# hmmlillian/Neural-Color-Transfer

Measured on AMD Instinct MI355X. Metric: 700x700 pairs/sec end-to-end L=5->1; PatchMatch HBM GB/s vs peak, higher is better.
Workload: dtype f32

## Files before the change

### neural-color-transfer_amd/csrc/k_s1.hip

```cpp
#include "nct_internal.h"
#include "nct_device.h"
#include "nct_reduce.h"
#include <cstdlib>
#include <rocprim/device/device_radix_sort.hpp>
#include <rocprim/device/device_scan.hpp>

#define LAB_D(u) ((double)(u) * (1.0 / 255.0))
#define LCHK() NCT_LAUNCH_CHECK()

constexpr int S1_SEG = NCT_S1_SEG;

struct S1Sys {
    int n, h, w;
    const double *daa, *dab, *dbb;
    const double *gx, *gy;
    const int* knn_id;
    nct_s1_graph g;
    int xcd;
    int one_xcd;
};
__device__ __forceinline__ int s1_one_xcd(int bid, int sel) { return (bid & 7) == sel - 1 ? (bid >> 3) : -1; }
__device__ __forceinline__ int s1_block_of(int bid, int nblocks, int xcd) {
    if (!xcd) return bid;
    const int q = nblocks >> 3, r = nblocks & 7, x = bid & 7, idx = bid >> 3;
    return (x < r ? x * (q + 1) : r * (q + 1) + (x - r) * q) + idx;
}
struct S1State { double gm[3], al[3], be[3]; int active[3], iters[3]; };

__device__ __forceinline__ void ld6(const double* __restrict__ v, size_t px, double (&o)[6]) {
    const double2* q = reinterpret_cast<const double2*>(v + px * 6);
    const double2 t0 = q[0], t1 = q[1], t2 = q[2];
    o[0] = t0.x; o[1] = t0.y; o[2] = t1.x; o[3] = t1.y; o[4] = t2.x; o[5] = t2.y;
}
__device__ __forceinline__ void st6(double* __restrict__ v, size_t px, const double (&o)[6]) {
    double2* q = reinterpret_cast<double2*>(v + px * 6);
    q[0] = make_double2(o[0], o[1]); q[1] = make_double2(o[2], o[3]); q[2] = make_double2(o[4], o[5]);
}
__device__ __forceinline__ int lo32(unsigned long long v) { return (int)(unsigned)(v & 0xFFFFFFFFull); }
__device__ __forceinline__ int hi32(unsigned long long v) { return (int)(unsigned)(v >> 32); }

__global__ void k_s1_iw2(const double* __restrict__ knn_w, int m, double nonlocalWeight, double* __restrict__ iw2) {
    const int e = blockIdx.x * blockDim.x + threadIdx.x;
    if (e >= m) return;
    const double iw = sqrt(knn_w[e]) * nonlocalWeight;
    iw2[e] = iw * iw;
}
__global__ void k_edge_keys(const int* __restrict__ knn_id, int m, unsigned* __restrict__ keys, unsigned* __restrict__ vals) {
    const int e = blockIdx.x * blockDim.x + threadIdx.x;
    if (e >= m) return;
    keys[e] = (unsigned)knn_id[e]; vals[e] = (unsigned)e;
}
__global__ void k_seg_starts(const unsigned* __restrict__ keys, int m, int* __restrict__ start, int n) {
    const int s = blockIdx.x * blockDim.x + threadIdx.x;
    if (s > n) return;
    int lo = 0, hi = m;
    while (lo < hi) { const int mid = (lo + hi) >> 1; if (keys[mid] < (unsigned)s) lo = mid + 1; else hi = mid; }
    start[s] = lo;
}
__global__ void k_s1_counts(const int* __restrict__ rev_start, int n, unsigned long long* __restrict__ cnt) {
    const int i = blockIdx.x * blockDim.x + threadIdx.x;
    if (i > n) return;
    unsigned long long v = 0;
    if (i < n) {
        const int deg = rev_start[i + 1] - rev_start[i];
        v = (unsigned long long)(deg < S1_SEG ? deg : S1_SEG) | ((unsigned long long)(deg > S1_SEG ? (deg - 1) / S1_SEG : 0) << 32);
    }
    cnt[i] = v;
}
__global__ void k_s1_sup_counts(const unsigned long long* __restrict__ starts, int n, int* __restrict__ cnt) {
    const int i = blockIdx.x * blockDim.x + threadIdx.x;
    if (i > n) return;
    int c = 0;
    if (i < n) { const int m = hi32(starts[i + 1]) - hi32(starts[i]); c = m > S1_SEG ? (m + S1_SEG - 1) / S1_SEG : 0; }
    cnt[i] = c;
}
__global__ void k_s1_sup_fill(const unsigned long long* __restrict__ starts, const int* __restrict__ sup_start, int n, int* __restrict__ sup_b0) {
    const int i = blockIdx.x * blockDim.x + threadIdx.x;
    if (i >= n) return;
    const int s0 = sup_start[i], ns = sup_start[i + 1] - s0, b0 = hi32(starts[i]);
    for (int k = 0; k < ns; ++k) sup_b0[s0 + k] = b0 + k * S1_SEG;
}
__global__ void k_s1_rev_build(const unsigned* __restrict__ keys_sorted, const unsigned* __restrict__ edge_sorted, const double* __restrict__ iw2, int m,
                               const int* __restrict__ rev_start, const unsigned long long* __restrict__ starts,
                               int* __restrict__ c_src, double* __restrict__ c_w, int* __restrict__ rev_src, double* __restrict__ rev_w,
                               int* __restrict__ seg_tgt, int* __restrict__ seg_e0) {
    const int e = blockIdx.x * blockDim.x + threadIdx.x;
    if (e >= m) return;
    const int t = (int)keys_sorted[e];
    const int rank = e - rev_start[t];
    const unsigned ed = edge_sorted[e];
    const int src = (int)(ed >> 3); const double wt = iw2[ed];
    const unsigned long long st = starts[t];
    if (rank < S1_SEG) { const int pos = lo32(st) + rank; c_src[pos] = src; c_w[pos] = wt; }
    else {
        rev_src[e] = src; rev_w[e] = wt;
        if ((rank & (S1_SEG - 1)) == 0) { const int sg = hi32(st) + rank / S1_SEG - 1; seg_tgt[sg] = t; seg_e0[sg] = e; }
    }
}

int nctk_s1_graph_build(nct_ctx* ctx, hipStream_t s, const int* knn_id, const double* knn_w, double nonlocalWeight, const nct_s1_graph& g, int* nseg_pinned) {
    const int n = g.n, m = 8 * n;
    DevBuf<unsigned> ek(ctx, m), ev(ctx, m), eks(ctx, m), evs(ctx, m);
    DevBuf<unsigned long long> cnt(ctx, (size_t)n + 1);
    DevBuf<int> scnt(ctx, (size_t)n + 1);
    if (!ek.ok() || !ev.ok() || !eks.ok() || !evs.ok() || !cnt.ok() || !scnt.ok()) return NCT_ERR_HIP;
    hipLaunchKernelGGL(k_s1_iw2, dim3(cdiv(m, 256)), dim3(256), 0, s, knn_w, m, nonlocalWeight, g.iw2); LCHK();
    hipLaunchKernelGGL(k_edge_keys, dim3(cdiv(m, 256)), dim3(256), 0, s, knn_id, m, (unsigned*)ek, (unsigned*)ev); LCHK();
    int end_bit = 1; while ((1u << end_bit) < (unsigned)n && end_bit < 32) ++end_bit;
    size_t tmp_bytes = 0, scan_bytes = 0, scan2_bytes = 0;
    NCT_HIP(rocprim::radix_sort_pairs(nullptr, tmp_bytes, (const unsigned*)ek, (unsigned*)eks, (const unsigned*)ev, (unsigned*)evs, m, 0, end_bit, s));
    NCT_HIP(rocprim::exclusive_scan(nullptr, scan_bytes, (const unsigned long long*)cnt, g.starts, 0ull, (size_t)n + 1, rocprim::plus<unsigned long long>(), s));
    NCT_HIP(rocprim::exclusive_scan(nullptr, scan2_bytes, (const int*)scnt, g.sup_start, 0, (size_t)n + 1, rocprim::plus<int>(), s));
    if (scan2_bytes > scan_bytes) scan_bytes = scan2_bytes;
    DevBuf<char> tmp(ctx, (tmp_bytes > scan_bytes ? tmp_bytes : scan_bytes) + 16);
    if (!tmp.ok()) return NCT_ERR_HIP;
    NCT_HIP(rocprim::radix_sort_pairs((void*)(char*)tmp, tmp_bytes, (const unsigned*)ek, (unsigned*)eks, (const unsigned*)ev, (unsigned*)evs, m, 0, end_bit, s));
    hipLaunchKernelGGL(k_seg_starts, dim3(cdiv(n + 1, 256)), dim3(256), 0, s, (const unsigned*)eks, m, g.rev_start, n); LCHK();
    hipLaunchKernelGGL(k_s1_counts, dim3(cdiv(n + 1, 256)), dim3(256), 0, s, (const int*)g.rev_start, n, (unsigned long long*)cnt); LCHK();
    NCT_HIP(rocprim::exclusive_scan((void*)(char*)tmp, scan_bytes, (const unsigned long long*)cnt, g.starts, 0ull, (size_t)n + 1, rocprim::plus<unsigned long long>(), s));
    hipLaunchKernelGGL(k_s1_rev_build, dim3(cdiv(m, 256)), dim3(256), 0, s, (const unsigned*)eks, (const unsigned*)evs, (const double*)g.iw2, m, (const int*)g.rev_start,
                       (const unsigned long long*)g.starts, g.c_src, g.c_w, g.rev_src, g.rev_w, g.seg_tgt, g.seg_e0); LCHK();
    hipLaunchKernelGGL(k_s1_sup_counts, dim3(cdiv(n + 1, 256)), dim3(256), 0, s, (const unsigned long long*)g.starts, n, (int*)scnt); LCHK();
    NCT_HIP(rocprim::exclusive_scan((void*)(char*)tmp, scan2_bytes, (const int*)scnt, g.sup_start, 0, (size_t)n + 1, rocprim::plus<int>(), s));
    hipLaunchKernelGGL(k_s1_sup_fill, dim3(cdiv(n, 256)), dim3(256), 0, s, (const unsigned long long*)g.starts, (const int*)g.sup_start, n, g.sup_b0); LCHK();
    if (nseg_pinned) {
        NCT_HIP(hipMemcpyAsync(nseg_pinned, (const char*)(g.starts + n) + 4, sizeof(int), hipMemcpyDeviceToHost, s));
        NCT_HIP(hipMemcpyAsync(nseg_pinned + 1, g.sup_start + n, sizeof(int), hipMemcpyDeviceToHost, s));
    }
    return 0;
}

__global__ void k_s1_setup(int n, const double* __restrict__ weight, float dWeight, const uint8_t* __restrict__ src, const uint8_t* __restrict__ ref,
                           double* __restrict__ daa, double* __restrict__ dab, double* __restrict__ dbb, double* __restrict__ rhs ) {
    const int i = blockIdx.x * blockDim.x + threadIdx.x;
    if (i >= n) return;
    const double dw = sqrt(weight[i]) * (double)sqrtf(dWeight);
#pragma unroll
    for (int c = 0; c < 3; ++c) {
        const double v0 = dw * LAB_D(src[(size_t)i * 3 + c]);
        const double rb = dw * LAB_D(ref[(size_t)i * 3 + c]);
        daa[(size_t)i * 3 + c] = v0 * v0; dab[(size_t)i * 3 + c] = v0 * dw; dbb[(size_t)i * 3 + c] = dw * dw;
        rhs[(size_t)i * 3 + c] = v0 * rb; rhs[(size_t)(n + i) * 3 + c] = dw * rb;
    }
}

__global__ __launch_bounds__(256) void k_s1_hub(nct_s1_graph G, const double* __restrict__ v ) {
    const int nseg = hi32(G.starts[G.n]);
    const int lane = threadIdx.x & 63;
    for (int sg = blockIdx.x * 4 + (threadIdx.x >> 6); sg < nseg; sg += gridDim.x * 4) {
        const int t = G.seg_tgt[sg];
        const int e = G.seg_e0[sg] + lane;
        const bool in = e < G.rev_start[t + 1];
        double term[6], vt[6], vj[6];
        int j = t; double wt = 0.0;
        if (in) { j = G.rev_src[e]; wt = G.rev_w[e]; }
        ld6(v, (size_t)t, vt); ld6(v, (size_t)j, vj);
#pragma unroll
        for (int c = 0; c < 6; ++c) { const double d = wt * (vt[c] - vj[c]); term[c] = in ? d : 0.0; }
#pragma unroll
        for (int off = 32; off >= 1; off >>= 1)
#pragma unroll
            for (int c = 0; c < 6; ++c) term[c] += __shfl_xor(term[c], off);
        if (lane == 0) {
#pragma unroll
            for (int c = 0; c < 6; ++c) G.hub_part[(size_t)sg * 6 + c] = term[c];
        }
    }
}

__global__ __launch_bounds__(256) void k_s1_hub2(nct_s1_graph G) {
    const int nsup = G.sup_start[G.n];
    const int lane = threadIdx.x & 63;
    for (int sb = blockIdx.x * 4 + (threadIdx.x >> 6); sb < nsup; sb += gridDim.x * 4) {
        const int b0 = G.sup_b0[sb];
        const int t = G.seg_tgt[b0];
        const int bend = min(b0 + S1_SEG, hi32(G.starts[t + 1]));
        double term[6];
        const bool in = b0 + lane < bend;
        if (in) ld6(G.hub_part, (size_t)(b0 + lane), term);
#pragma unroll
        for (int c = 0; c < 6; ++c) term[c] = in ? term[c] : 0.0;
#pragma unroll
        for (int off = 32; off >= 1; off >>= 1)
#pragma unroll
            for (int c = 0; c < 6; ++c) term[c] += __shfl_xor(term[c], off);
        if (lane == 0) st6(G.sup_part, (size_t)sb, term);
    }
}

#ifndef NCT_S1_CHUNK
#define NCT_S1_CHUNK 1024
#endif
constexpr int S1_CHUNK = NCT_S1_CHUNK;
template <bool COOP>
__device__ __forceinline__ void s1_op(const S1Sys& S, const double* __restrict__ p, int i, bool live, double (&a)[3], double (&b)[3], double (&ya)[3], double (&yb)[3], int lb = -1) {
    const int w = S.w, h = S.h;
    int e0 = 0, e1 = 0, h0 = 0, h1 = 0;
#pragma unroll
    for (int c = 0; c < 3; ++c) { a[c] = 0.0; b[c] = 0.0; ya[c] = 0.0; yb[c] = 0.0; }
    if (live) {
        const int y = i / w, x = i - y * w;
        { double own[6]; ld6(p, (size_t)i, own);
#pragma unroll
          for (int c = 0; c < 3; ++c) { a[c] = own[c]; b[c] = own[3 + c]; } }
#pragma unroll
        for (int c = 0; c < 3; ++c) {
            ya[c] = S.daa[(size_t)i * 3 + c] * a[c] + S.dab[(size_t)i * 3 + c] * b[c];
            yb[c] = S.dab[(size_t)i * 3 + c] * a[c] + S.dbb[(size_t)i * 3 + c] * b[c];
        }
        auto edge = [&](int j, double wt) {
            double q[6]; ld6(p, (size_t)j, q);
#pragma unroll
            for (int c = 0; c < 3; ++c) { ya[c] += wt * (a[c] - q[c]); yb[c] += wt * (b[c] - q[3 + c]); }
        };
        {
            const bool ex[4] = {x + 1 < w, x > 0, y + 1 < h, y > 0};
            const int nj[4] = {ex[0] ? i + 1 : i, ex[1] ? i - 1 : i, ex[2] ? i + w : i, ex[3] ? i - w : i};
            const double g4[4] = {S.gx[i], S.gx[ex[1] ? i - 1 : i], S.gy[i], S.gy[ex[3] ? i - w : i]};
            double q4[4][6];
#pragma unroll
            for (int u = 0; u < 4; ++u) ld6(p, (size_t)nj[u], q4[u]);
#pragma unroll
            for (int u = 0; u < 4; ++u)
                if (ex[u]) {
                    const double wt = 2.0 * (g4[u] * g4[u]);
#pragma unroll
                    for (int c = 0; c < 3; ++c) { ya[c] += wt * (a[c] - q4[u][c]); yb[c] += wt * (b[c] - q4[u][3 + c]); }
                }
        }
#pragma unroll
        for (int k = 0; k < 8; ++k) edge(S.knn_id[(size_t)i * 8 + k], S.g.iw2[(size_t)i * 8 + k]);
        const unsigned long long s0 = S.g.starts[i], s1 = S.g.starts[i + 1];
        e0 = lo32(s0); e1 = lo32(s1); h0 = hi32(s0); h1 = hi32(s1);
    }
    if constexpr (!COOP) {
        if (live) {
            int e = e0;
            for (; e + 4 <= e1; e += 4) {
                int j[4]; double wt[4], pv[4][6];
#pragma unroll
                for (int u = 0; u < 4; ++u) { j[u] = S.g.c_src[e + u]; wt[u] = S.g.c_w[e + u]; }
#pragma unroll
                for (int u = 0; u < 4; ++u) ld6(p, (size_t)j[u], pv[u]);
#pragma unroll
                for (int u = 0; u < 4; ++u)
#pragma unroll
                    for (int c = 0; c < 3; ++c) { ya[c] += wt[u] * (a[c] - pv[u][c]); yb[c] += wt[u] * (b[c] - pv[u][3 + c]); }
            }
            for (; e < e1; ++e) {
                const int j = S.g.c_src[e]; const double wt = S.g.c_w[e];
                double q[6]; ld6(p, (size_t)j, q);
#pragma unroll
                for (int c = 0; c < 3; ++c) { ya[c] += wt * (a[c] - q[c]); yb[c] += wt * (b[c] - q[3 + c]); }
            }
        }
    } else {
        __shared__ double s_pv[6 * S1_CHUNK];
        __shared__ double s_wt[S1_CHUNK];
        const int i0 = (lb >= 0 ? lb : (int)blockIdx.x) * 256, i1 = min(i0 + 256, S.n);
        const int E0 = lo32(S.g.starts[i0]), E1 = lo32(S.g.starts[i1]);
        for (int base = E0; base < E1; base += S1_CHUNK) {
            const int cnt = min(S1_CHUNK, E1 - base);
            for (int t = threadIdx.x; t < cnt; t += 256) {
                const int j = S.g.c_src[base + t];
                s_wt[t] = S.g.c_w[base + t];
                double q[6]; ld6(p, (size_t)j, q);
#pragma unroll
                for (int c = 0; c < 6; ++c) s_pv[c * S1_CHUNK + t] = q[c];
            }
            __syncthreads();
            const int lo = max(e0, base) - base, hi = min(e1, base + cnt) - base;
            for (int t = lo; t < hi; ++t) {
                const double wt = s_wt[t];
#pragma unroll
                for (int c = 0; c < 3; ++c) { ya[c] += wt * (a[c] - s_pv[c * S1_CHUNK + t]); yb[c] += wt * (b[c] - s_pv[(3 + c) * S1_CHUNK + t]); }
            }
            __syncthreads();
        }
    }
    bool sup = false;
    if (h1 - h0 > S1_SEG) { h0 = S.g.sup_start[i]; h1 = S.g.sup_start[i + 1]; sup = true; }
    const double* __restrict__ part = sup ? S.g.sup_part : S.g.hub_part;
    for (int sg = h0; sg < h1; ++sg) {
        double q[6]; ld6(part, (size_t)sg, q);
#pragma unroll
        for (int c = 0; c < 3; ++c) { ya[c] += q[c]; yb[c] += q[3 + c]; }
    }
}

template <bool COOP>
__global__ __launch_bounds__(256) void k_s1_residual(S1Sys S, const double* __restrict__ x6, const double* __restrict__ rhs, double* __restrict__ r6) {
    const int i = blockIdx.x * 256 + threadIdx.x;
    double a[3], b[3], ya[3], yb[3];
    s1_op<COOP>(S, x6, i, i < S.n, a, b, ya, yb);
    if (i < S.n) {
        double o[6];
#pragma unroll
        for (int c = 0; c < 3; ++c) { o[c] = rhs[(size_t)i * 3 + c] - ya[c]; o[3 + c] = rhs[(size_t)(S.n + i) * 3 + c] - yb[c]; }
        st6(r6, (size_t)i, o);
    }
}
template <bool COOP>
__global__ __launch_bounds__(256) void k_s1_apply(S1Sys S, const double* __restrict__ r6, double* __restrict__ w6, double* __restrict__ partial ) {
    const int lb = S.one_xcd ? s1_one_xcd(blockIdx.x, S.one_xcd) : s1_block_of(blockIdx.x, gridDim.x, S.xcd);
    if (lb < 0) return;
    const int i = lb * 256 + threadIdx.x;
    double acc[6] = {0, 0, 0, 0, 0, 0};
    double a[3], b[3], ya[3], yb[3];
    s1_op<COOP>(S, r6, i, i < S.n, a, b, ya, yb, lb);
    if (i < S.n) {
#pragma unroll
        for (int c = 0; c < 3; ++c) {
            acc[c] = a[c] * a[c] + b[c] * b[c];
            acc[3 + c] = a[c] * ya[c] + b[c] * yb[c];
        }
        const double o[6] = {ya[0], ya[1], ya[2], yb[0], yb[1], yb[2]};
        st6(w6, (size_t)i, o);
    }
    block_reduce_store<6>(acc, partial, lb);
}

__device__ __forceinline__ void s1_scalars(bool first, const double (&sm)[6], const S1State* __restrict__ in, double tol2, S1State& o) {
#pragma unroll
    for (int c = 0; c < 3; ++c) {
        if (first) {
            const double g0 = sm[c]; const bool act = g0 > tol2;
            o.gm[c] = g0; o.be[c] = 0.0; o.al[c] = act ? g0 / sm[3 + c] : 0.0; o.active[c] = act ? 1 : 0; o.iters[c] = act ? 1 : 0;
        } else if (in->active[c]) {
            const double g1 = sm[c];
            const double be = g1 / in->gm[c];
            const double al = g1 / (sm[3 + c] - (be * g1) / in->al[c]);
            const bool act = g1 > tol2;
            o.gm[c] = g1; o.be[c] = be; o.al[c] = al; o.active[c] = act ? 1 : 0; o.iters[c] = in->iters[c] + (act ? 1 : 0);
        } else {
            o.gm[c] = in->gm[c]; o.be[c] = in->be[c]; o.al[c] = in->al[c]; o.active[c] = 0; o.iters[c] = in->iters[c];
        }
    }
}
__global__ __launch_bounds__(256) void k_s1_scal(const double* __restrict__ partial, int nb, const S1State* __restrict__ in, S1State* __restrict__ out, int first, double tol2) {
    double sm[6]; final_reduce<6>(partial, nb, sm);
    if (threadIdx.x == 0) { S1State o; s1_scalars(first != 0, sm, in, tol2, o); *out = o; }
}
constexpr int S1_FUSE_NB = 512;
template <bool FUSED>
__global__ __launch_bounds__(256) void k_s1_update(int n, int nb, const double* __restrict__ partial, const S1State* __restrict__ sin, S1State* __restrict__ sout,
                                                   int first_scal, double tol2, int first_vec, double* __restrict__ r6, const double* __restrict__ w6,
                                                   double* __restrict__ p6, double* __restrict__ s6, double* __restrict__ x6, int one_xcd) {
    const int bid = one_xcd ? s1_one_xcd(blockIdx.x, one_xcd) : (int)blockIdx.x;
    if (bid < 0) return;
    const size_t total = (size_t)3 * n;
    const size_t base = (size_t)bid * 768 + threadIdx.x;
    double2 rv[3], wv[3], pv[3], sv[3], xv[3];
    const double2* r2 = reinterpret_cast<const double2*>(r6); const double2* w2 = reinterpret_cast<const double2*>(w6);
    const double2* x2 = reinterpret_cast<const double2*>(x6); const double2* p2 = reinterpret_cast<const double2*>(p6); const double2* s2 = reinterpret_cast<const double2*>(s6);
#pragma unroll
    for (int k = 0; k < 3; ++k) {
        const size_t g0 = base + (size_t)k * 256, g = g0 < total ? g0 : total - 1;
        rv[k] = r2[g]; wv[k] = w2[g]; xv[k] = x2[g];
        pv[k] = p2[g]; sv[k] = s2[g];
        if (first_vec) { pv[k] = make_double2(0.0, 0.0); sv[k] = make_double2(0.0, 0.0); }
    }
    double al[3], be[3]; bool act[3];
    if constexpr (FUSED) {
        double sm[6]; final_reduce<6>(partial, nb, sm);
        S1State o; s1_scalars(first_scal != 0, sm, sin, tol2, o);
        if (bid == 0 && threadIdx.x == 0) *sout = o;
#pragma unroll
        for (int c = 0; c < 3; ++c) { al[c] = o.al[c]; be[c] = o.be[c]; act[c] = o.active[c] != 0; }
    } else {
#pragma unroll
        for (int c = 0; c < 3; ++c) { al[c] = sin->al[c]; be[c] = sin->be[c]; act[c] = sin->active[c] != 0; }
    }
    double2* r2o = reinterpret_cast<double2*>(r6); double2* x2o = reinterpret_cast<double2*>(x6); double2* p2o = reinterpret_cast<double2*>(p6); double2* s2o = reinterpret_cast<double2*>(s6);
#pragma unroll
    for (int k = 0; k < 3; ++k) {
        const size_t g = base + (size_t)k * 256;
        if (g >= total) continue;
        const int c0 = (int)((2 * g) % 3), c1 = (c0 + 1) % 3;
        const double a0 = c0 == 0 ? al[0] : (c0 == 1 ? al[1] : al[2]), b0 = c0 == 0 ? be[0] : (c0 == 1 ? be[1] : be[2]);
        const double a1 = c1 == 0 ? al[0] : (c1 == 1 ? al[1] : al[2]), b1 = c1 == 0 ? be[0] : (c1 == 1 ? be[1] : be[2]);
        const bool on0 = c0 == 0 ? act[0] : (c0 == 1 ? act[1] : act[2]), on1 = c1 == 0 ? act[0] : (c1 == 1 ? act[1] : act[2]);
        double2 pn, sn, xn, rn;
        pn.x = first_vec ? rv[k].x : b0 * pv[k].x + rv[k].x;  pn.y = first_vec ? rv[k].y : b1 * pv[k].y + rv[k].y;
        sn.x = first_vec ? wv[k].x : b0 * sv[k].x + wv[k].x;  sn.y = first_vec ? wv[k].y : b1 * sv[k].y + wv[k].y;
        xn.x = xv[k].x + a0 * pn.x;  xn.y = xv[k].y + a1 * pn.y;
        rn.x = rv[k].x - a0 * sn.x;  rn.y = rv[k].y - a1 * sn.y;
        if (!on0) { pn.x = pv[k].x; sn.x = sv[k].x; xn.x = xv[k].x; rn.x = rv[k].x; }
        if (!on1) { pn.y = pv[k].y; sn.y = sv[k].y; xn.y = xv[k].y; rn.y = rv[k].y; }
        if (on0 || on1) { p2o[g] = pn; s2o[g] = sn; x2o[g] = xn; r2o[g] = rn; }
    }
}
__global__ void k_pack6(int n, const double* __restrict__ x, double* __restrict__ x6) {
    const int i = blockIdx.x * blockDim.x + threadIdx.x;
    if (i >= 2 * n * 3) return;
    const int c = i % 3, part = i / (n * 3), px = (i - part * n * 3) / 3;
    x6[(size_t)px * 6 + part * 3 + c] = x[i];
}
__global__ void k_unpack6(int n, const double* __restrict__ x6, double* __restrict__ x) {
    const int i = blockIdx.x * blockDim.x + threadIdx.x;
    if (i >= 2 * n * 3) return;
    const int c = i % 3, part = i / (n * 3), px = (i - part * n * 3) / 3;
    x[i] = x6[(size_t)px * 6 + part * 3 + c];
}

int nctk_s1_solve(nct_ctx* ctx, hipStream_t s, const nct_s1_graph& g, const int* knn_id, const double* weight, float dWeight, const uint8_t* s_lab_level,
                  const uint8_t* g_lab_level, const double* gx, const double* gy, int layer, int h, int w, double* x, int* cg_iters_host ) {
    const int n = h * w, nbl = cdiv(n, 256);
    DevBuf<double> daa(ctx, (size_t)3 * n), dab(ctx, (size_t)3 * n), dbb(ctx, (size_t)3 * n), rhs(ctx, (size_t)6 * n);
    DevBuf<double> x6(ctx, (size_t)6 * n), r6(ctx, (size_t)6 * n), w6(ctx, (size_t)6 * n), p6(ctx, (size_t)6 * n), s6(ctx, (size_t)6 * n), partial(ctx, (size_t)nbl * 6);
    DevBuf<S1State> st(ctx, 2);
    if (!daa.ok() || !dab.ok() || !dbb.ok() || !rhs.ok() || !x6.ok() || !r6.ok() || !w6.ok() || !p6.ok() || !s6.ok() || !partial.ok() || !st.ok()) return NCT_ERR_HIP;
    hipLaunchKernelGGL(k_s1_setup, dim3(nbl), dim3(256), 0, s, n, weight, dWeight, s_lab_level, g_lab_level, (double*)daa, (double*)dab, (double*)dbb, (double*)rhs); LCHK();
    static const int s1_xcd = [] { const char* e = getenv("NCT_S1_XCD"); return e ? atoi(e) : 1; }();
    static const int s1_one_max = [] { const char* e = getenv("NCT_S1_ONE_XCD_MAX"); return e ? atoi(e) : 32; }();
    const int one_xcd = (nbl <= s1_one_max && nbl <= S1_FUSE_NB) ? 1 + (ctx->home_xcd & 7) : 0;
    const int ogrid = one_xcd ? nbl * 8 : nbl;
    S1Sys S{n, h, w, daa, dab, dbb, gx, gy, knn_id, g, (s1_xcd && n >= 100000) ? 1 : 0, one_xcd};
    const double tol2 = 1e-6 * 1e-6;
    const int maxit = layer == 4 ? 50 : 100;
    const bool coop = n >= 100000;
    const bool fused = nbl <= S1_FUSE_NB;
    const int hub_blind = cdiv(cdiv(8 * n, S1_SEG), 4) < 256 ? cdiv(cdiv(8 * n, S1_SEG), 4) : 256;
    const int hub_grid = g.nseg_hint == 0 ? 0 : (g.nseg_hint > 0 ? (cdiv(g.nseg_hint, 4) < 4096 ? cdiv(g.nseg_hint, 4) : 4096) : hub_blind);
    const int hub2_grid = (g.nseg_hint == 0 || g.nsup_hint == 0) ? 0 : (g.nsup_hint > 0 ? (cdiv(g.nsup_hint, 4) < 1024 ? cdiv(g.nsup_hint, 4) : 1024) : (cdiv(hub_blind, S1_SEG) < 64 ? cdiv(hub_blind, S1_SEG) : 64));
    auto hub = [&](const double* v) -> int {
        if (hub_grid) { hipLaunchKernelGGL(k_s1_hub, dim3(hub_grid), dim3(256), 0, s, g, v); LCHK(); }
        if (hub2_grid) { hipLaunchKernelGGL(k_s1_hub2, dim3(hub2_grid), dim3(256), 0, s, g); LCHK(); }
        return 0;
    };
    auto apply = [&](bool kt) -> int {
        if (kt) { int rk = ctx->kt_begin(s, NCT_KT_S1_APPLY); if (rk) return rk; }
        if (coop) hipLaunchKernelGGL(k_s1_apply<true>, dim3(nbl), dim3(256), 0, s, S, (const double*)r6, (double*)w6, (double*)partial);
        else      hipLaunchKernelGGL(k_s1_apply<false>, dim3(ogrid), dim3(256), 0, s, S, (const double*)r6, (double*)w6, (double*)partial);
        LCHK();
        if (kt) { int rk = ctx->kt_end(s); if (rk) return rk; }
        return 0;
    };
    hipLaunchKernelGGL(k_pack6, dim3(cdiv(6 * n, 256)), dim3(256), 0, s, n, (const double*)x, (double*)x6); LCHK();
    { int rc = hub(x6); if (rc) return rc; }
    if (coop) hipLaunchKernelGGL(k_s1_residual<true>, dim3(nbl), dim3(256), 0, s, S, (const double*)x6, (const double*)rhs, (double*)r6);
    else      hipLaunchKernelGGL(k_s1_residual<false>, dim3(nbl), dim3(256), 0, s, S, (const double*)x6, (const double*)rhs, (double*)r6);
    LCHK();
    { int rc = hub(r6); if (rc) return rc; rc = apply(false); if (rc) return rc; }
    S1State* slot[2] = {(S1State*)st, (S1State*)st + 1};
    for (int k = 1; k <= maxit; ++k) {
        const bool kt = ctx->kt_on && layer == 4 && k >= 3 && k < 11;
        if (fused) {
            hipLaunchKernelGGL(k_s1_update<true>, dim3(ogrid), dim3(256), 0, s, n, nbl, (const double*)partial, (const S1State*)slot[k & 1], slot[(k - 1) & 1], k == 1 ? 1 : 0, tol2,
                               k == 1 ? 1 : 0, (double*)r6, (const double*)w6, (double*)p6, (double*)s6, (double*)x6, one_xcd); LCHK();
        } else {
            if (kt) { int rk = ctx->kt_begin(s, NCT_KT_S1_SCALARS); if (rk) return rk; }
            hipLaunchKernelGGL(k_s1_scal, dim3(1), dim3(256), 0, s, (const double*)partial, nbl, (const S1State*)slot[k & 1], slot[(k - 1) & 1], k == 1 ? 1 : 0, tol2); LCHK();
            if (kt) { int rk = ctx->kt_end(s); if (rk) return rk; rk = ctx->kt_begin(s, NCT_KT_S1_UPDATE); if (rk) return rk; }
            hipLaunchKernelGGL(k_s1_update<false>, dim3(nbl), dim3(256), 0, s, n, nbl, (const double*)partial, (const S1State*)slot[(k - 1) & 1], slot[(k - 1) & 1], 0, tol2,
                               k == 1 ? 1 : 0, (double*)r6, (const double*)w6, (double*)p6, (double*)s6, (double*)x6, 0); LCHK();
            if (kt) { int rk = ctx->kt_end(s); if (rk) return rk; }
        }
        if (k < maxit) { int rc = hub(r6); if (rc) return rc; rc = apply(kt); if (rc) return rc; }
    }
    hipLaunchKernelGGL(k_unpack6, dim3(cdiv(6 * n, 256)), dim3(256), 0, s, n, (const double*)x6, x); LCHK();
    if (cg_iters_host) {
        S1State hst;
        NCT_HIP(hipMemcpyAsync(&hst, slot[(maxit - 1) & 1], sizeof hst, hipMemcpyDeviceToHost, s));
        NCT_HIP(hipStreamSynchronize(s));
        for (int c = 0; c < 3; ++c) cg_iters_host[c] = hst.iters[c];
    }
    return 0;
}
```

### neural-color-transfer_amd/csrc/nct_internal.h

```cpp
#pragma once
#include <hip/hip_runtime.h>
#include <cstdint>
#include <cstdio>
#include <cstdarg>
#include <string>
#include <vector>
#include "../../include/nct.h"

struct nct_block { void* p; size_t bytes; bool used; };

struct nct_ctx {
    int device = 0;
    hipStream_t stream = nullptr;
    hipStream_t stream2 = nullptr;
    hipEvent_t ev0 = nullptr, ev1 = nullptr, ev_fork = nullptr, ev_join = nullptr;
    hipEvent_t ev_level[5] = {nullptr, nullptr, nullptr, nullptr, nullptr};
    hipEvent_t ev_poll[4] = {nullptr, nullptr, nullptr, nullptr};
    hipStream_t stream_wls = nullptr;
    hipEvent_t ev_wls_fork = nullptr, ev_wls_join = nullptr;
    void* pinned = nullptr;
    std::string err;
    std::vector<nct_block> blocks;
    size_t bytes_allocated = 0;
    float *bench_a = nullptr, *bench_b = nullptr; void *bench_ah16 = nullptr, *bench_bh16 = nullptr; int bench_C = 0, bench_ah = 0, bench_aw = 0, bench_bh = 0, bench_bw = 0;
    void* vgg = nullptr;
    void* cvt = nullptr;
    void* pair = nullptr;
    unsigned long long* d_counter = nullptr;
    int home_xcd = 0;
    int pm_persist = 0;
    int pm_persist_wgs = 0;
    uint32_t* d_pm_err = nullptr;
    unsigned pm_attr_mask = 0;
    int wls_split = 0;
    int wls_forecast = 1;
    int wls_lines = 1;
    int wls_graph = 0;
    int conv_pool_fuse = -1;
    double wls_rtol = 3e-8;
    int wls_maxit = 5000;
    bool tm_on = false;
    std::vector<hipEvent_t> tm_events;
    std::vector<double> tm_host;
    std::vector<int> tm_tags;
    int mark(hipStream_t s, int tag);
    int conv_pair = 1;
    int* s1_hub_blocks() { return (int*)((char*)pinned + 4096); }
    long long s1_hub_blocks_last[5] = {0, 0, 0, 0, 0};
    int knn_runs = -1;
    int s1_hub_hint = 1;
    int s1_hub_wait = 1;
    bool kt_on = false;
    std::vector<hipEvent_t> kt_events; std::vector<int> kt_ids;
    int kt_begin(hipStream_t s, int id);
    int kt_end(hipStream_t s);

    int fail(int code, const char* fmt, ...) {
        char buf[512]; va_list ap; va_start(ap, fmt); vsnprintf(buf, sizeof buf, fmt, ap); va_end(ap);
        err = buf; return code;
    }
    void* alloc(size_t bytes);
    void release(void* p);
    bool defer_release = false;
    std::vector<void*> deferred;
    void flush_deferred() { for (void* p : deferred) for (auto& b : blocks) if (b.p == p) { b.used = false; break; } deferred.clear(); }
};

template <typename T> struct DevBuf {
    nct_ctx* c; T* p;
    DevBuf(nct_ctx* ctx, size_t n) : c(ctx), p((T*)ctx->alloc(n * sizeof(T))) {}
    ~DevBuf() { if (p) c->release(p); }
    DevBuf(const DevBuf&) = delete; DevBuf& operator=(const DevBuf&) = delete;
    operator T*() const { return p; }
    bool ok() const { return p != nullptr; }
};

#define NCT_HIP(call) do { hipError_t e_ = (call); if (e_ != hipSuccess) \
    return ctx->fail(NCT_ERR_HIP, "%s failed: %s (%s:%d)", #call, hipGetErrorString(e_), __FILE__, __LINE__); } while (0)
#define NCT_LAUNCH_CHECK() NCT_HIP(hipGetLastError())
#define NCT_REQUIRE(cond, ...) do { if (!(cond)) return ctx->fail(NCT_ERR_INVALID, __VA_ARGS__); } while (0)

static inline int cdiv(int a, int b) { return (a + b - 1) / b; }

int nctk_chw_to_hwc(nct_ctx* ctx, hipStream_t s, const float* src, float* dst, int C, int HW);
int nctk_hwc_to_chw(nct_ctx* ctx, hipStream_t s, const float* src, float* dst, int C, int HW);
int nctk_normalize(nct_ctx* ctx, hipStream_t s, const float* src_hwc, float* dst_hwc, float* resp , int C, int HW,
                   void* dst_h16 = nullptr );
int nctk_feature_distance(nct_ctx* ctx, hipStream_t s, const float* a_hwc, const float* b_hwc, float* err, int C, int HW);
int nctk_pm_check(nct_ctx* ctx);
int nctk_nnf_init(nct_ctx* ctx, hipStream_t s, uint32_t* nnf, int ah, int aw, int bh, int bw);
int nctk_nnf_upsample(nct_ctx* ctx, hipStream_t s, const uint32_t* nnf_half, uint32_t* nnf, int ah, int aw, int bh, int bw, int ah_half, int aw_half);
int nctk_patchmatch(nct_ctx* ctx, hipStream_t s, const float* a_hwc, const float* b_hwc, int C, int ah, int aw, int bh, int bw,
                    int iters, int rs_max, uint32_t seed, uint32_t* nnf, float* dist, unsigned long long* eval_counter );
int nctk_conv3x3_pair(nct_ctx* ctx, hipStream_t s, const float* in1, int H1, int W1, const float* in2, int H2, int W2, const float* wp, const float* bias,
                      float* out1, float* out2, int Cin, int Cout, int relu, float* hwc1, float* hwc2);
int nctk_vgg19_forward_pair(nct_ctx* ctx, hipStream_t s, const uint8_t* d_bgr1, int H1, int W1, int stride1, float* const* taps_hwc1,
                            const uint8_t* d_bgr2, int H2, int W2, int stride2, float* const* taps_hwc2);
int nctk_vgg19_forward(nct_ctx* ctx, hipStream_t s, const uint8_t* d_bgr, int H, int W, int stride, int deepest_tap, float* const* d_taps_chw, int* dims,
                       float* const* d_taps_hwc = nullptr );
void nct_vgg_free(nct_ctx* ctx);
int nctk_bgr2lab(nct_ctx* ctx, hipStream_t s, const uint8_t* src, uint8_t* dst, size_t npix);
int nctk_lab2bgr(nct_ctx* ctx, hipStream_t s, const uint8_t* src, uint8_t* dst, size_t npix, int form = 0 );
int nctk_resize_u8c3(nct_ctx* ctx, hipStream_t s, const uint8_t* src, int sh, int sw, uint8_t* dst, int dh, int dw);
int nctk_resize_f64c3(nct_ctx* ctx, hipStream_t s, const double* src, int sh, int sw, double* dst, int dh, int dw);
void nct_cvt_free(nct_ctx* ctx);
void nct_pair_free(nct_ctx* ctx);
int nct_stage_tag_nonlocal(); int nct_stage_tag_wls(); int nct_stage_tag_color();
int nctk_kmeans_labels(nct_ctx* ctx, hipStream_t s, const float* feat_hwc_norm, int n, int C, int K, int iters, uint64_t seed, int* labels, int* nlabels_dev);
int nctk_knn_graph(nct_ctx* ctx, hipStream_t s, const uint8_t* lab_u8, int h, int w, const int* labels, int lh, int lw, int nlabels, const int* nlabels_dev , int samples,
                   int* knn_id, double* knn_w);
#define NCT_S1_SEG 64
struct nct_s1_graph {
    int n;
    double* iw2;
    unsigned long long* starts;
    int* c_src; double* c_w;
    int* rev_start;
    int* rev_src; double* rev_w;
    int* seg_tgt; int* seg_e0;
    double* hub_part;
    int* sup_start;
    int* sup_b0;
    double* sup_part;
    int nseg_hint, nsup_hint;
};
struct nct_s1_graph_bufs {
    int n;
    DevBuf<double> iw2, c_w, rev_w, hub_part, sup_part; DevBuf<unsigned long long> starts; DevBuf<int> c_src, rev_start, rev_src, seg_tgt, seg_e0, sup_start, sup_b0;
    nct_s1_graph_bufs(nct_ctx* c, int n_) : n(n_), iw2(c, (size_t)8 * n_), c_w(c, (size_t)8 * n_), rev_w(c, (size_t)8 * n_), hub_part(c, ((size_t)n_ / 8 + 1) * 6), sup_part(c, ((size_t)n_ / 256 + 2) * 6),
                                            starts(c, (size_t)n_ + 1), c_src(c, (size_t)8 * n_), rev_start(c, (size_t)n_ + 1), rev_src(c, (size_t)8 * n_), seg_tgt(c, (size_t)n_ / 8 + 1),
                                            seg_e0(c, (size_t)n_ / 8 + 1), sup_start(c, (size_t)n_ + 1), sup_b0(c, (size_t)n_ / 256 + 2) {}
    bool ok() const { return iw2.ok() && c_w.ok() && rev_w.ok() && hub_part.ok() && sup_part.ok() && starts.ok() && c_src.ok() && rev_start.ok() && rev_src.ok() && seg_tgt.ok() && seg_e0.ok() && sup_start.ok() && sup_b0.ok(); }
    nct_s1_graph view(int hint, int hint2) const { return nct_s1_graph{n, iw2, starts, c_src, c_w, rev_start, rev_src, rev_w, seg_tgt, seg_e0, hub_part, sup_start, sup_b0, sup_part, hint, hint2}; }
};
int nctk_s1_graph_build(nct_ctx* ctx, hipStream_t s, const int* knn_id, const double* knn_w, double nonlocalWeight, const nct_s1_graph& g, int* nseg_pinned );
int nctk_s1_solve(nct_ctx* ctx, hipStream_t s, const nct_s1_graph& g, const int* knn_id, const double* weight, float dWeight, const uint8_t* s_lab_level,
                  const uint8_t* g_lab_level, const double* gx, const double* gy, int layer, int h, int w, double* x, int* cg_iters_host);
struct nct_color_params { double eps, nonlocal_weight, local_weight, wls_lambda_init, wls_alpha, k_num; };
struct nct_color_debug { double *ab_local, *ab_nonlocal, *ab_up, *rough, *ab_wls; int* cg_iters; int* wls_iters; };
int nctk_local_color_transfer(nct_ctx* ctx, hipStream_t s, const float* err, const uint8_t* s_lab_level, const uint8_t* g_lab_level,
                              const uint8_t* s_lab_full, const int* knn_id, const double* knn_w, int layer, int h, int w, int H, int W,
                              const nct_color_params& prm, uint8_t* out_lab_full, const nct_color_debug* dbg,
                              const nct_s1_graph* graph = nullptr );
int nctk_wls_solve_mg(nct_ctx* ctx, hipStream_t s, double* X, const double* rough, const double* wx, const double* wy, int H, int W,
                      double rtol, int* iters_out);
enum { NCT_PM_PLAIN = 0,
       NCT_PM_ROWREJECT = 1,
       NCT_PM_FP16 = 2 };
int nctk_patchmatch_bidir(nct_ctx* ctx, hipStream_t s, const float* a_hwc, const float* b_hwc, const void* a_h16, const void* b_h16, int C, int ah, int aw, int bh, int bw,
                          int iters, int rs_max, uint32_t seed_ab, uint32_t seed_ba, uint32_t* ann, float* annd, uint32_t* bnn, float* bnnd,
                          int pm_mode, unsigned long long* counters );
int nctk_bds_vote_features(nct_ctx* ctx, hipStream_t s, const uint32_t* ann, const uint32_t* bnn, const float* pin_hwc, float* pout_hwc, float* pw ,
                           int C, int ah, int aw, int bh, int bw, float w_coh, float w_comp);
int nctk_bds_vote_image(nct_ctx* ctx, hipStream_t s, const uint8_t* b_bgr, const uint32_t* ann, const uint32_t* bnn,
                        int ah, int aw, int bh, int bw, double w_coh, double w_comp, uint8_t* out_bgr);
int nctk_bds_vote_both(nct_ctx* ctx, hipStream_t s, const uint8_t* b_bgr, const float* pin_hwc, const uint32_t* ann, const uint32_t* bnn, int C,
                       int ah, int aw, int bh, int bw, double w_coh, double w_comp, uint8_t* out_bgr, float* pout_hwc);
```

Baseline: 14.72.

## Reuse LDS-staged reverse-edge values for mutual kNN forward edges in S1 operator

At graph-build time a per-forward-edge slot map (mslot) is recorded, storing where each kNN neighbour also appears in the node's reverse-edge list. In the cooperative S1 matvec, forward kNN edges whose partner value is already being staged into shared memory for the reverse-edge pass read it from LDS instead of doing a scattered global 6-double load. Accumulation of those forward edges is deferred until the matching chunk is resident. This adds a memset and a small extra pass in graph build, plus register pressure from the eight deferred 6-double operands held across the chunk loop.

```diff
diff --git a/neural-color-transfer_amd/csrc/k_s1.hip b/neural-color-transfer_amd/csrc/k_s1.hip
--- a/neural-color-transfer_amd/csrc/k_s1.hip
+++ b/neural-color-transfer_amd/csrc/k_s1.hip
@@ -18,6 +18,7 @@
     nct_s1_graph g;
     int xcd;
     int one_xcd;
+    int mutual;
 };
 __device__ __forceinline__ int s1_one_xcd(int bid, int sel) { return (bid & 7) == sel - 1 ? (bid >> 3) : -1; }
 __device__ __forceinline__ int s1_block_of(int bid, int nblocks, int xcd) {
@@ -81,9 +82,9 @@
     for (int k = 0; k < ns; ++k) sup_b0[s0 + k] = b0 + k * S1_SEG;
 }
 __global__ void k_s1_rev_build(const unsigned* __restrict__ keys_sorted, const unsigned* __restrict__ edge_sorted, const double* __restrict__ iw2, int m,
-                               const int* __restrict__ rev_start, const unsigned long long* __restrict__ starts,
+                               const int* __restrict__ rev_start, const unsigned long long* __restrict__ starts, const int* __restrict__ knn_id,
                                int* __restrict__ c_src, double* __restrict__ c_w, int* __restrict__ rev_src, double* __restrict__ rev_w,
-                               int* __restrict__ seg_tgt, int* __restrict__ seg_e0) {
+                               int* __restrict__ seg_tgt, int* __restrict__ seg_e0, uint8_t* __restrict__ mslot) {
     const int e = blockIdx.x * blockDim.x + threadIdx.x;
     if (e >= m) return;
     const int t = (int)keys_sorted[e];
@@ -91,7 +92,15 @@
     const unsigned ed = edge_sorted[e];
     const int src = (int)(ed >> 3); const double wt = iw2[ed];
     const unsigned long long st = starts[t];
-    if (rank < S1_SEG) { const int pos = lo32(st) + rank; c_src[pos] = src; c_w[pos] = wt; }
+    if (rank < S1_SEG) {
+        const int pos = lo32(st) + rank; c_src[pos] = src; c_w[pos] = wt;
+        int ids[8];
+#pragma unroll
+        for (int k = 0; k < 8; ++k) ids[k] = knn_id[(size_t)t * 8 + k];
+#pragma unroll
+        for (int k = 0; k < 8; ++k)
+            if (ids[k] == src) mslot[(size_t)t * 8 + k] = (uint8_t)rank;
+    }
     else {
         rev_src[e] = src; rev_w[e] = wt;
         if ((rank & (S1_SEG - 1)) == 0) { const int sg = hi32(st) + rank / S1_SEG - 1; seg_tgt[sg] = t; seg_e0[sg] = e; }
@@ -118,8 +127,9 @@
     hipLaunchKernelGGL(k_seg_starts, dim3(cdiv(n + 1, 256)), dim3(256), 0, s, (const unsigned*)eks, m, g.rev_start, n); LCHK();
     hipLaunchKernelGGL(k_s1_counts, dim3(cdiv(n + 1, 256)), dim3(256), 0, s, (const int*)g.rev_start, n, (unsigned long long*)cnt); LCHK();
     NCT_HIP(rocprim::exclusive_scan((void*)(char*)tmp, scan_bytes, (const unsigned long long*)cnt, g.starts, 0ull, (size_t)n + 1, rocprim::plus<unsigned long long>(), s));
+    NCT_HIP(hipMemsetAsync(g.mslot, 0xFF, (size_t)m, s));
     hipLaunchKernelGGL(k_s1_rev_build, dim3(cdiv(m, 256)), dim3(256), 0, s, (const unsigned*)eks, (const unsigned*)evs, (const double*)g.iw2, m, (const int*)g.rev_start,
-                       (const unsigned long long*)g.starts, g.c_src, g.c_w, g.rev_src, g.rev_w, g.seg_tgt, g.seg_e0); LCHK();
+                       (const unsigned long long*)g.starts, knn_id, g.c_src, g.c_w, g.rev_src, g.rev_w, g.seg_tgt, g.seg_e0, g.mslot); LCHK();
     hipLaunchKernelGGL(k_s1_sup_counts, dim3(cdiv(n + 1, 256)), dim3(256), 0, s, (const unsigned long long*)g.starts, n, (int*)scnt); LCHK();
     NCT_HIP(rocprim::exclusive_scan((void*)(char*)tmp, scan2_bytes, (const int*)scnt, g.sup_start, 0, (size_t)n + 1, rocprim::plus<int>(), s));
     hipLaunchKernelGGL(k_s1_sup_fill, dim3(cdiv(n, 256)), dim3(256), 0, s, (const unsigned long long*)g.starts, (const int*)g.sup_start, n, g.sup_b0); LCHK();
@@ -196,10 +206,20 @@
 __device__ __forceinline__ void s1_op(const S1Sys& S, const double* __restrict__ p, int i, bool live, double (&a)[3], double (&b)[3], double (&ya)[3], double (&yb)[3], int lb = -1) {
     const int w = S.w, h = S.h;
     int e0 = 0, e1 = 0, h0 = 0, h1 = 0;
+    int E0 = 0, E1 = 0;
+    int ok_lds = 0, lds_t[8];
+    double ow[8], oq[8][6];
+    bool pending = false;
+    if constexpr (COOP) {
+        const int i0 = (lb >= 0 ? lb : (int)blockIdx.x) * 256, i1 = min(i0 + 256, S.n);
+        E0 = lo32(S.g.starts[i0]); E1 = lo32(S.g.starts[i1]);
+    }
 #pragma unroll
     for (int c = 0; c < 3; ++c) { a[c] = 0.0; b[c] = 0.0; ya[c] = 0.0; yb[c] = 0.0; }
     if (live) {
         const int y = i / w, x = i - y * w;
+        const unsigned long long s0 = S.g.starts[i], s1 = S.g.starts[i + 1];
+        e0 = lo32(s0); e1 = lo32(s1); h0 = hi32(s0); h1 = hi32(s1);
         { double own[6]; ld6(p, (size_t)i, own);
 #pragma unroll
           for (int c = 0; c < 3; ++c) { a[c] = own[c]; b[c] = own[3 + c]; } }
@@ -213,6 +233,22 @@
 #pragma unroll
             for (int c = 0; c < 3; ++c) { ya[c] += wt * (a[c] - q[c]); yb[c] += wt * (b[c] - q[3 + c]); }
         };
+        if constexpr (COOP) {
+            unsigned long long ms = ~0ull;
+            if (S.mutual) ms = *reinterpret_cast<const unsigned long long*>(S.g.mslot + (size_t)i * 8);
+            const int cb = E0 + ((e0 - E0) / S1_CHUNK) * S1_CHUNK;
+#pragma unroll
+            for (int k = 0; k < 8; ++k) {
+                const int j = S.knn_id[(size_t)i * 8 + k];
+                ow[k] = S.g.iw2[(size_t)i * 8 + k];
+                const int sl = (int)((ms >> (8 * k)) & 0xFF);
+                const bool in_lds = sl != 0xFF && e0 + sl < cb + S1_CHUNK;
+                lds_t[k] = in_lds ? e0 + sl - cb : 0;
+                ok_lds |= in_lds ? 1 << k : 0;
+                ld6(p, (size_t)(in_lds ? i : j), oq[k]);
+            }
+            pending = S.mutual != 0;
+        }
         {
             const bool ex[4] = {x + 1 < w, x > 0, y + 1 < h, y > 0};
             const int nj[4] = {ex[0] ? i + 1 : i, ex[1] ? i - 1 : i, ex[2] ? i + w : i, ex[3] ? i - w : i};
@@ -228,10 +264,15 @@
                     for (int c = 0; c < 3; ++c) { ya[c] += wt * (a[c] - q4[u][c]); yb[c] += wt * (b[c] - q4[u][3 + c]); }
                 }
         }
-#pragma unroll
-        for (int k = 0; k < 8; ++k) edge(S.knn_id[(size_t)i * 8 + k], S.g.iw2[(size_t)i * 8 + k]);
-        const unsigned long long s0 = S.g.starts[i], s1 = S.g.starts[i + 1];
-        e0 = lo32(s0); e1 = lo32(s1); h0 = hi32(s0); h1 = hi32(s1);
+        if constexpr (!COOP) {
+#pragma unroll
+            for (int k = 0; k < 8; ++k) edge(S.knn_id[(size_t)i * 8 + k], S.g.iw2[(size_t)i * 8 + k]);
+        } else if (!pending) {
+#pragma unroll
+            for (int k = 0; k < 8; ++k)
+#pragma unroll
+                for (int c = 0; c < 3; ++c) { ya[c] += ow[k] * (a[c] - oq[k][c]); yb[c] += ow[k] * (b[c] - oq[k][3 + c]); }
+        }
     }
     if constexpr (!COOP) {
         if (live) {
@@ -257,8 +298,6 @@
     } else {
         __shared__ double s_pv[6 * S1_CHUNK];
         __shared__ double s_wt[S1_CHUNK];
-        const int i0 = (lb >= 0 ? lb : (int)blockIdx.x) * 256, i1 = min(i0 + 256, S.n);
-        const int E0 = lo32(S.g.starts[i0]), E1 = lo32(S.g.starts[i1]);
         for (int base = E0; base < E1; base += S1_CHUNK) {
             const int cnt = min(S1_CHUNK, E1 - base);
             for (int t = threadIdx.x; t < cnt; t += 256) {
@@ -269,6 +308,19 @@
                 for (int c = 0; c < 6; ++c) s_pv[c * S1_CHUNK + t] = q[c];
             }
             __syncthreads();
+            if (pending && e0 < base + cnt) {
+#pragma unroll
+                for (int k = 0; k < 8; ++k) {
+                    const bool in_lds = (ok_lds >> k) & 1;
+#pragma unroll
+                    for (int c = 0; c < 3; ++c) {
+                        const double qa = in_lds ? s_pv[c * S1_CHUNK + lds_t[k]] : oq[k][c];
+                        const double qb = in_lds ? s_pv[(3 + c) * S1_CHUNK + lds_t[k]] : oq[k][3 + c];
+                        ya[c] += ow[k] * (a[c] - qa); yb[c] += ow[k] * (b[c] - qb);
+                    }
+                }
+                pending = false;
+            }
             const int lo = max(e0, base) - base, hi = min(e1, base + cnt) - base;
             for (int t = lo; t < hi; ++t) {
                 const double wt = s_wt[t];
@@ -276,6 +328,12 @@
                 for (int c = 0; c < 3; ++c) { ya[c] += wt * (a[c] - s_pv[c * S1_CHUNK + t]); yb[c] += wt * (b[c] - s_pv[(3 + c) * S1_CHUNK + t]); }
             }
             __syncthreads();
+        }
+        if (pending) {
+#pragma unroll
+            for (int k = 0; k < 8; ++k)
+#pragma unroll
+                for (int c = 0; c < 3; ++c) { ya[c] += ow[k] * (a[c] - oq[k][c]); yb[c] += ow[k] * (b[c] - oq[k][3 + c]); }
         }
     }
     bool sup = false;
@@ -413,9 +471,10 @@
     hipLaunchKernelGGL(k_s1_setup, dim3(nbl), dim3(256), 0, s, n, weight, dWeight, s_lab_level, g_lab_level, (double*)daa, (double*)dab, (double*)dbb, (double*)rhs); LCHK();
     static const int s1_xcd = [] { const char* e = getenv("NCT_S1_XCD"); return e ? atoi(e) : 1; }();
     static const int s1_one_max = [] { const char* e = getenv("NCT_S1_ONE_XCD_MAX"); return e ? atoi(e) : 32; }();
+    static const int s1_mutual = [] { const char* e = getenv("NCT_S1_MUTUAL"); return e ? atoi(e) : 1; }();
     const int one_xcd = (nbl <= s1_one_max && nbl <= S1_FUSE_NB) ? 1 + (ctx->home_xcd & 7) : 0;
     const int ogrid = one_xcd ? nbl * 8 : nbl;
-    S1Sys S{n, h, w, daa, dab, dbb, gx, gy, knn_id, g, (s1_xcd && n >= 100000) ? 1 : 0, one_xcd};
+    S1Sys S{n, h, w, daa, dab, dbb, gx, gy, knn_id, g, (s1_xcd && n >= 100000) ? 1 : 0, one_xcd, s1_mutual ? 1 : 0};
     const double tol2 = 1e-6 * 1e-6;
     const int maxit = layer == 4 ? 50 : 100;
     const bool coop = n >= 100000;
diff --git a/neural-color-transfer_amd/csrc/nct_internal.h b/neural-color-transfer_amd/csrc/nct_internal.h
--- a/neural-color-transfer_amd/csrc/nct_internal.h
+++ b/neural-color-transfer_amd/csrc/nct_internal.h
@@ -122,16 +122,17 @@
     int* sup_start;
     int* sup_b0;
     double* sup_part;
+    uint8_t* mslot;
     int nseg_hint, nsup_hint;
 };
 struct nct_s1_graph_bufs {
     int n;
-    DevBuf<double> iw2, c_w, rev_w, hub_part, sup_part; DevBuf<unsigned long long> starts; DevBuf<int> c_src, rev_start, rev_src, seg_tgt, seg_e0, sup_start, sup_b0;
+    DevBuf<double> iw2, c_w, rev_w, hub_part, sup_part; DevBuf<unsigned long long> starts; DevBuf<int> c_src, rev_start, rev_src, seg_tgt, seg_e0, sup_start, sup_b0; DevBuf<uint8_t> mslot;
     nct_s1_graph_bufs(nct_ctx* c, int n_) : n(n_), iw2(c, (size_t)8 * n_), c_w(c, (size_t)8 * n_), rev_w(c, (size_t)8 * n_), hub_part(c, ((size_t)n_ / 8 + 1) * 6), sup_part(c, ((size_t)n_ / 256 + 2) * 6),
                                             starts(c, (size_t)n_ + 1), c_src(c, (size_t)8 * n_), rev_start(c, (size_t)n_ + 1), rev_src(c, (size_t)8 * n_), seg_tgt(c, (size_t)n_ / 8 + 1),
-                                            seg_e0(c, (size_t)n_ / 8 + 1), sup_start(c, (size_t)n_ + 1), sup_b0(c, (size_t)n_ / 256 + 2) {}
-    bool ok() const { return iw2.ok() && c_w.ok() && rev_w.ok() && hub_part.ok() && sup_part.ok() && starts.ok() && c_src.ok() && rev_start.ok() && rev_src.ok() && seg_tgt.ok() && seg_e0.ok() && sup_start.ok() && sup_b0.ok(); }
-    nct_s1_graph view(int hint, int hint2) const { return nct_s1_graph{n, iw2, starts, c_src, c_w, rev_start, rev_src, rev_w, seg_tgt, seg_e0, hub_part, sup_start, sup_b0, sup_part, hint, hint2}; }
+                                            seg_e0(c, (size_t)n_ / 8 + 1), sup_start(c, (size_t)n_ + 1), sup_b0(c, (size_t)n_ / 256 + 2), mslot(c, (size_t)8 * n_) {}
+    bool ok() const { return iw2.ok() && c_w.ok() && rev_w.ok() && hub_part.ok() && sup_part.ok() && starts.ok() && c_src.ok() && rev_start.ok() && rev_src.ok() && seg_tgt.ok() && seg_e0.ok() && sup_start.ok() && sup_b0.ok() && mslot.ok(); }
+    nct_s1_graph view(int hint, int hint2) const { return nct_s1_graph{n, iw2, starts, c_src, c_w, rev_start, rev_src, rev_w, seg_tgt, seg_e0, hub_part, sup_start, sup_b0, sup_part, mslot, hint, hint2}; }
 };
 int nctk_s1_graph_build(nct_ctx* ctx, hipStream_t s, const int* knn_id, const double* knn_w, double nonlocalWeight, const nct_s1_graph& g, int* nseg_pinned );
 int nctk_s1_solve(nct_ctx* ctx, hipStream_t s, const nct_s1_graph& g, const int* knn_id, const double* weight, float dWeight, const uint8_t* s_lab_level,
```

Measured after the change: 14.98 (median of 6 runs). 1.02x the previous value.
